# K-Kielak/dopamine

Measured on AMD Instinct MI355X. Metric: gradient-steps/sec (Rainbow, batch=32, 1M-transition buffer), higher is better.
Workload: dtype fp32; 1 GPU; Rainbow/C51 Asterix (9 actions), prioritized sum-tree replay, n=3, 1M-transition 84x84x4 uint8 buffer per GPU; global_batch=32, per_gpu_batch=32, replay_capacity=1000000, parallelism=dp1, hip_graph=True

## Files before the change

### dopamine_amd/csrc/nature_cnn.hip

```cpp
#include <algorithm>
#include <cassert>

#include "cnn_tile.h"
#include "c51_dev.h"

#include <cstring>
#include <optional>
#include <tuple>
#include <type_traits>

namespace dq {
namespace cnn {

constexpr int kGroupT = 1024;

template <int WM, int WN, int WK, class AL, class BL, class EP, bool kLate = true, int KS = 0,
          int NS = 0>
struct GemmOp {
  static constexpr int kT = 64 * WM * WN * WK;
  static constexpr bool kLateFetch = kLate;
  static constexpr int kLds = Tile<WM, WN, WK>::template lds<AL, BL>();
  AL a;
  BL b;
  EP e;
// ... 1240 lines not shown
  const int nc = std::max(kPubBlocks, blocks_for(P.lo, 2));
  const int na = blocks_for((P.n - P.lo) * (P.world - 1) / P.world, 4);
  auto rd = [&](int i) { return i >= 1 && i - 1 < n_riders ? riders + (i - 1) : nullptr; };
  launch(c, rd(1), b.dX_fc1());
  launch(c, rd(2), b.dW_fc1(), b.dX_c3(), b.dW_fc2());
  launch(c, rd(3), PeerPubOp{P, kPeerGrad}, b.dW_c3(), b.subpix_pairs(), b.dW_c2(), rs(s0, sm));
  launch(c, rd(4), b.sum_c3(), b.dW_c1(), rs(sm, s1));
  const PeerAgOp ag = defer_ag ? AgParts{&P, oa->var}.head()
                               : PeerAgOp{P, oa->var, na, 0, 0, INT64_MAX};
  launch(c, rd(5), PeerPubOp{P, kPeerParam}, b.sum_c2(), b.sum_c1(),
         P.world > 1 ? std::optional(ag) : std::nullopt);
  launch(c, NoRider{}, PeerExchOp{P, od, oa->var, oa->m, oa->v, nc}, head_layer<0>(head));
}

template <int kOpt>
void backward_head_from(Ctx& c, const dq_cnn_params* p, const dq_cnn_params* g, int B,
                        const float* x, const dq_cnn_acts* a, const float* dout, dq_cnn_acts* d,
                        const AdamHost& opt, int first, int last, const RiderDesc* r, int n_riders,
                        const FwdOps* hp, int head_from) {
  if (head_from == 7)
    backward_grouped<kOpt, 5>(c, p, g, B, x, a, dout, d, opt, first, last, r, n_riders, nullptr);
  else if (head_from == 6)
    backward_grouped<kOpt, 6>(c, p, g, B, x, a, dout, d, opt, first, last, r, n_riders, hp);
  else if (head_from == 5)
    backward_grouped<kOpt, 5>(c, p, g, B, x, a, dout, d, opt, first, last, r, n_riders, hp);
  else if (head_from == 4)
    backward_grouped<kOpt, 4>(c, p, g, B, x, a, dout, d, opt, first, last, r, n_riders, hp);
  else
    backward_grouped<kOpt>(c, p, g, B, x, a, dout, d, opt, first, last, r, n_riders, hp);
}

}
}

using namespace dq;
using namespace dq::cnn;

static int check_adam(const dq_cnn_params* p, const dq_cnn_params* g, const dq_adam_args* opt) {
  DQ_CHECK_ARG(opt->kind == DQ_OPT_ADAM || opt->kind == DQ_OPT_RMSPROP, "unknown optimizer kind");
  if (opt->kind == DQ_OPT_ADAM)
    DQ_CHECK_ARG(opt->var && opt->m && opt->v && opt->state && (opt->slot == 0 || opt->slot == 1),
                 "adam args: var, m, v, state and slot 0/1 required");
  else
    DQ_CHECK_ARG(opt->var && opt->m && opt->v && (!opt->centered || opt->mg),
                 "rmsprop args: var, ms (m), mom (v) and, centered, mg required");
  const float* w[10] = {p->conv1_w, p->conv1_b, p->conv2_w, p->conv2_b, p->conv3_w,
                        p->conv3_b, p->fc1_w,  p->fc1_b,  p->fc2_w,  p->fc2_b};
  const float* gw[10] = {g->conv1_w, g->conv1_b, g->conv2_w, g->conv2_b, g->conv3_w,
                         g->conv3_b, g->fc1_w,  g->fc1_b,  g->fc2_w,  g->fc2_b};
  for (int i = 0; i < 10; ++i) {
    DQ_CHECK_ARG(w[i] >= opt->var && (i == 0 || w[i] > w[i - 1]),
                 "parameters must live in the flat buffer opt->var in conv1..fc2 order");
    DQ_CHECK_ARG(gw[i] - g->conv1_w == w[i] - p->conv1_w,
                 "gradients must have the parameters' flat layout");
  }
  DQ_CHECK_ARG(((p->conv2_w - opt->var) & 3) == 0 && ((g->conv2_w - g->conv1_w) & 3) == 0,
               "16-byte aligned parameter views required");
  return DQ_OK;
}

#define DQ_TRY(expr)                   \
  do {                                 \
    const int rc_ = (expr);            \
    if (rc_ != DQ_OK) return rc_;      \
  } while (0)

static int check_net(bool args, int32_t batch, const dq_cnn_params* p, bool fc = true) {
  DQ_CHECK_ARG(args && batch >= 1, "null argument");
  DQ_CHECK_ARG(p->in_channels == 4 && (!fc || p->n_out >= 1),
               "the Nature CNN takes 84x84x4 NHWC input");
  return DQ_OK;
}
static int check_nets(bool args, int32_t batch, const dq_cnn_params* p0, const dq_cnn_params* p1,
                      const float* ws0, const float* ws1) {
  DQ_CHECK_ARG(args && batch >= 1, "null argument");
  DQ_CHECK_ARG(p0->in_channels == 4 && p1->in_channels == 4 && p0->n_out >= 1 && p1->n_out >= 1,
               "the Nature CNN takes 84x84x4 NHWC input");
  DQ_CHECK_ARG(ws0 != ws1, "the two networks need separate workspaces");
  return DQ_OK;
}
static int copy_riders(const dq_rider* riders, int32_t n_riders, int most, const char* too_many,
                       RiderDesc* r) {
  DQ_CHECK_ARG(0 <= n_riders && n_riders <= most && (riders || n_riders == 0), too_many);
  for (int i = 0; i < n_riders; ++i) {
    memcpy(&r[i], &riders[i], sizeof(RiderDesc));
    DQ_CHECK_ARG(r[i].kind >= kRiderNone && r[i].kind <= kRiderSetSample, "corrupt rider");
  }
  return DQ_OK;
}
static int head_ops(const dq_cnn_net* head, const float* ws, int32_t batch, FwdOps* hf,
                    const FwdOps** hp) {
  *hp = nullptr;
  if (!head) return DQ_OK;
  DQ_CHECK_ARG(head->p && head->x && head->a && head->ws, "null head network field");
  DQ_CHECK_ARG(head->p->in_channels == 4, "the Nature CNN takes 84x84x4 NHWC input");
  DQ_CHECK_ARG(head->ws != ws, "the head network needs its own workspace");
  *hf = FwdOps{head->p, head->x, head->a, head->ws, batch};
  *hp = hf;
  return DQ_OK;
}

static int check_peer(const dq_peer* peer, const float* var) {
  DQ_CHECK_ARG(peer && var, "null argument");
  const dq_peer& P = *peer;
  DQ_CHECK_ARG(P.world >= 1 && P.world <= DQ_PEER_MAX && P.rank >= 0 && P.rank < P.world,
               "peer: 1 <= world <= DQ_PEER_MAX, 0 <= rank < world");
  DQ_CHECK_ARG(P.lo >= 0 && P.lo % 4 == 0 && P.n > P.lo && (P.n - P.lo) % (4 * P.world) == 0,
               "peer: lo % 4 == 0 and (n - lo) % (4 world) == 0");
  DQ_CHECK_ARG(P.param[P.rank] == var, "peer: var must be this rank's parameter buffer");
  for (int q = 0; q < P.world; ++q)
    DQ_CHECK_ARG(P.grad[q] && P.param[q] && P.flags[q], "peer: null rank buffer");
  DQ_CHECK_ARG(P.max_polls > 0, "peer: max_polls must be positive");
  DQ_CHECK_ARG(P.xcds >= 0 && P.xcds <= 8, "peer: 0 <= xcds <= 8");
  return DQ_OK;
}

extern "C" {

int dq_cnn_forward(const dq_cnn_params* p, int32_t batch, const float* x, dq_cnn_acts* a,
                   float* ws, void* stream) {
  DQ_TRY(check_net(p && a && x && ws, batch, p));
  Ctx c{(hipStream_t)stream, ws, false, 0};
  forward(c, p, batch, x, a);
  DQ_CHECK_LAUNCH("dq_cnn_forward");
  return DQ_OK;
}

int dq_cnn_forward_pair(const dq_cnn_params* p0, const float* x0, dq_cnn_acts* a0, float* ws0,
                        const dq_cnn_params* p1, const float* x1, dq_cnn_acts* a1, float* ws1,
                        int32_t batch, void* stream) {
  DQ_TRY(check_nets(p0 && a0 && x0 && ws0 && p1 && a1 && x1 && ws1, batch, p0, p1, ws0, ws1));
  Ctx c0{(hipStream_t)stream, ws0, false, 0}, c1{(hipStream_t)stream, ws1, false, 0};
  forward_pair(c0, c1, p0, x0, a0, p1, x1, a1, batch);
  DQ_CHECK_LAUNCH("dq_cnn_forward_pair");
  return DQ_OK;
}

int dq_cnn_forward_head(const dq_cnn_params* p, int32_t batch, const float* x, dq_cnn_acts* a,
                        float* ws, void* stream) {
  DQ_TRY(check_net(p && a && x && ws, batch, p));
  Ctx c{(hipStream_t)stream, ws, false, 0};
  forward_head(c, FwdOps{p, x, a, ws, batch});
  DQ_CHECK_LAUNCH("dq_cnn_forward_head");
  return DQ_OK;
}

int dq_cnn_forward_with_tail(const dq_cnn_params* p0, const float* x0, dq_cnn_acts* a0, float* ws0,
                             const dq_cnn_params* p1, dq_cnn_acts* a1, float* ws1, int32_t batch,
                             void* stream) {
  DQ_TRY(check_nets(p0 && a0 && x0 && ws0 && p1 && a1 && ws1, batch, p0, p1, ws0, ws1));
  Ctx c0{(hipStream_t)stream, ws0, false, 0}, c1{(hipStream_t)stream, ws1, false, 0};
  forward_with_tail(c0, c1, FwdOps{p0, x0, a0, ws0, batch}, FwdOps{p1, nullptr, a1, ws1, batch});
  DQ_CHECK_LAUNCH("dq_cnn_forward_with_tail");
  return DQ_OK;
}

int dq_cnn_forward_fused(const dq_cnn_params* p0, const float* x0, dq_cnn_acts* a0, float* ws0,
                         const dq_cnn_params* p1, const float* x1, dq_cnn_acts* a1, float* ws1,
                         int32_t batch, int32_t fc1_1, void* stream) {
  DQ_TRY(check_nets(p0 && a0 && x0 && ws0 && p1 && a1 && ws1, batch, p0, p1, ws0, ws1));
  Ctx c0{(hipStream_t)stream, ws0, false, 0}, c1{(hipStream_t)stream, ws1, false, 0};
  DQ_CHECK_ARG((fc1_1 & 12) != 12, "flags 4 (convs only) and 8 (fc layers only) exclude each other");
  DQ_CHECK_ARG(!(fc1_1 & 32) || x1, "flag 32 (net 1's conv1) needs x1");
  forward_fused(c0, c1, FwdOps{p0, x0, a0, ws0, batch}, FwdOps{p1, x1, a1, ws1, batch},
                (fc1_1 & 1) != 0, (fc1_1 & 2) != 0, (fc1_1 & 8) == 0, (fc1_1 & 4) == 0,
                (fc1_1 & 16) != 0, (fc1_1 & 32) != 0);
  DQ_CHECK_LAUNCH("dq_cnn_forward_fused");
  return DQ_OK;
}

size_t dq_cnn_fc2_parts_offset(int32_t batch) { return FwdOps::part_offset(batch); }

int dq_cnn_forward_fused_c51(const dq_cnn_params* p0, const float* x0, dq_cnn_acts* a0, float* ws0,
                             const dq_cnn_params* p1, dq_cnn_acts* a1, float* ws1, int32_t batch,
                             const dq_c51_target* c51, int32_t flags, void* stream) {
  DQ_TRY(check_nets(p0 && a0 && x0 && ws0 && p1 && a1 && ws1 && c51, batch, p0, p1, ws0, ws1));
  DQ_CHECK_ARG((flags & 12) != 12, "flags 4 (convs only) and 8 (fc layers only) exclude each other");
  DQ_CHECK_ARG(c51->rewards && c51->terminals && c51->support && c51->m_out, "null C51 argument");
  DQ_CHECK_ARG(c51->num_atoms >= 2 && c51->num_atoms <= 64 && p1->n_out % c51->num_atoms == 0,
               "n_out must be num_actions * num_atoms, 2 <= num_atoms <= 64");
  const int A = p1->n_out / c51->num_atoms;
  DQ_CHECK_ARG(A <= 4 * kC51TgtMaxWaveRows, "the riding C51 target half takes at most 16 actions");
  Ctx c0{(hipStream_t)stream, ws0, false, 0}, c1{(hipStream_t)stream, ws1, false, 0};
  const FwdOps f0{p0, x0, a0, ws0, batch}, f1{p1, nullptr, a1, ws1, batch};
  const int NO = p1->n_out;
  C51Target t{LogitsParts{ws1 + FwdOps::part_offset(batch), p1->fc2_b, (int64_t)batch * NO,
                          FcHeadOp::kBands, NO},
              c51->rewards, c51->terminals, c51->support, batch, A, c51->num_atoms,
              c51->cumulative_gamma, c51->m_out, c51->target_logits_out};
  forward_fused_c51(c0, c1, f0, f1, t, (flags & 8) == 0, (flags & 4) == 0);
  DQ_CHECK_LAUNCH("dq_cnn_forward_fused_c51");
  return DQ_OK;
}


int dq_cnn_backward(const dq_cnn_params* p, const dq_cnn_params* g, int32_t batch, const float* x,
                    const dq_cnn_acts* a, const float* dout, dq_cnn_acts* d, float* ws,
                    void* stream) {
  DQ_TRY(check_net(p && g && a && d && x && dout && ws, batch, p));
  Ctx c{(hipStream_t)stream, ws, false, 0};
  backward_grouped<0>(c, p, g, batch, x, a, dout, d, AdamHost{nullptr});
  DQ_CHECK_LAUNCH("dq_cnn_backward");
  return DQ_OK;
}

int dq_cnn_backward_adam(const dq_cnn_params* p, const dq_cnn_params* g, int32_t batch,
                         const float* x, const dq_cnn_acts* a, const float* dout, dq_cnn_acts* d,
                         float* ws, const dq_adam_args* opt, void* stream) {
  DQ_TRY(check_net(p && g && a && d && x && dout && ws && opt, batch, p));
  DQ_TRY(check_adam(p, g, opt));
  Ctx c{(hipStream_t)stream, ws, false, 0};
  if (opt->kind == DQ_OPT_RMSPROP)
    backward_grouped<2>(c, p, g, batch, x, a, dout, d, AdamHost{opt});
  else
    backward_grouped<1>(c, p, g, batch, x, a, dout, d, AdamHost{opt});
  DQ_CHECK_LAUNCH("dq_cnn_backward_adam");
  return DQ_OK;
}

int dq_cnn_backward_groups(const dq_cnn_params* p, const dq_cnn_params* g, int32_t batch,
                           const float* x, const dq_cnn_acts* a, const float* dout,
                           dq_cnn_acts* d, float* ws, int32_t first, int32_t last, void* stream) {
  DQ_TRY(check_net(p && g && a && d && x && dout && ws, batch, p));
  DQ_CHECK_ARG(0 <= first && first <= last && last <= 7, "groups must satisfy 0 <= first <= last <= 7");
  Ctx c{(hipStream_t)stream, ws, false, 0};
  backward_grouped<0>(c, p, g, batch, x, a, dout, d, AdamHost{nullptr}, first, last);
  DQ_CHECK_LAUNCH("dq_cnn_backward_groups");
  return DQ_OK;
}

int dq_cnn_backward_riders(const dq_cnn_params* p, const dq_cnn_params* g, int32_t batch,
                           const float* x, const dq_cnn_acts* a, const float* dout,
                           dq_cnn_acts* d, float* ws, const dq_rider* riders, int32_t n_riders,
                           const dq_adam_args* opt, const dq_cnn_net* head, int32_t head_from,
                           int32_t first, int32_t last, void* stream) {
  DQ_TRY(check_net(p && g && a && d && x && dout && ws, batch, p));
  RiderDesc r[7];
  DQ_TRY(copy_riders(riders, n_riders, 7, "at most one rider per grouped launch (7)", r));
  DQ_CHECK_ARG(0 <= first && first <= last && last <= 7, "groups must satisfy 0 <= first <= last <= 7");
  DQ_CHECK_ARG(!opt || (first <= 1 && last == 7), "the fused optimizer needs the whole backward");
  DQ_CHECK_ARG(head_from >= 3 && head_from <= 7, "head_from must be in [3, 7]");
  FwdOps hf{};
  const FwdOps* hp;
  DQ_TRY(head_ops(head, ws, batch, &hf, &hp));
  Ctx c{(hipStream_t)stream, ws, false, 0};
  if (opt) {
    DQ_TRY(check_adam(p, g, opt));
    if (opt->kind == DQ_OPT_RMSPROP)
      backward_head_from<2>(c, p, g, batch, x, a, dout, d, AdamHost{opt}, first, last, r, n_riders,
                            hp, head_from);
    else
      backward_head_from<1>(c, p, g, batch, x, a, dout, d, AdamHost{opt}, first, last, r, n_riders,
                            hp, head_from);
  } else {
    backward_head_from<0>(c, p, g, batch, x, a, dout, d, AdamHost{nullptr}, first, last, r,
                          n_riders, hp, head_from);
  }
  DQ_CHECK_LAUNCH("dq_cnn_backward_riders");
  return DQ_OK;
}

int dq_cnn_backward_peer(const dq_cnn_params* p, const dq_cnn_params* g, int32_t batch,
                         const float* x, const dq_cnn_acts* a, const float* dout,
                         dq_cnn_acts* d, float* ws, const dq_rider* riders, int32_t n_riders,
                         const dq_adam_args* opt, const dq_cnn_net* head, const dq_peer* peer,
                         int32_t defer_ag, void* stream) {
  DQ_TRY(check_net(p && g && a && d && x && dout && ws && opt && peer, batch, p));
  DQ_CHECK_ARG(opt->kind == DQ_OPT_ADAM, "the peer exchange applies TF1 Adam");
  RiderDesc r[5];
  DQ_TRY(copy_riders(riders, n_riders, 5, "at most one rider per grouped launch 1..5", r));
  DQ_TRY(check_adam(p, g, opt));
  DQ_TRY(check_peer(peer, opt->var));
  const dq_peer& P = *peer;
  DQ_CHECK_ARG(P.n >= (int64_t)(p->fc2_b + p->n_out - opt->var),
               "peer: [lo, n) must reach the end of the flat parameter buffer");
  DQ_CHECK_ARG(P.lo == (int64_t)(p->fc1_w - opt->var),
               "peer: the sharded range is exactly the fc bucket [fc1_w, n) (pad the flat buffer "
               "so that its length divides into 4 world-float slices)");
  DQ_CHECK_ARG(P.param[P.rank] == opt->var && P.grad[P.rank] == g->conv1_w - (p->conv1_w - opt->var),
               "peer: this rank's buffers must be opt->var and the gradient of its layout");
  FwdOps hf{};
  const FwdOps* hp;
  DQ_TRY(head_ops(head, ws, batch, &hf, &hp));
  Ctx c{(hipStream_t)stream, ws, false, 0};
  backward_peer(c, p, g, batch, x, a, dout, d, opt, r, n_riders, hp, P, defer_ag != 0);
  DQ_CHECK_LAUNCH("dq_cnn_backward_peer");
  return DQ_OK;
}

int dq_peer_all_gather(const dq_peer* peer, float* var, void* stream) {
  DQ_TRY(check_peer(peer, var));
  const dq_peer& P = *peer;
  if (P.world > 1) {
    Ctx c{(hipStream_t)stream, nullptr, false, 0};
    group(c, AgParts{peer, var}.part(0), AgParts{peer, var}.part(1), AgParts{peer, var}.part(2));
  }
  DQ_CHECK_LAUNCH("dq_peer_all_gather");
  return DQ_OK;
}

#ifdef DQ_GROUP_PROF
int dq_debug_group_reset(void) {
  static unsigned z[dq::cnn::kGrpPos];
  return hipMemcpyToSymbol(HIP_SYMBOL(dq::cnn::g_grp_seq), z, sizeof(z)) == hipSuccess ? 0 : -1;
}
int dq_debug_peer_phases(void* recs, unsigned* seq) {
  if (hipMemcpyFromSymbol(seq, HIP_SYMBOL(dq::cnn::g_peer_ph_seq), sizeof(dq::cnn::g_peer_ph_seq)) !=
      hipSuccess)
    return -1;
  return hipMemcpyFromSymbol(recs, HIP_SYMBOL(dq::cnn::g_peer_ph), sizeof(dq::cnn::g_peer_ph)) ==
                 hipSuccess ? 0 : -1;
}
int dq_debug_group_read(void* recs, unsigned* seq, unsigned* dims) {
  dims[0] = dq::cnn::kGrpPos;
  dims[1] = dq::cnn::kGrpRing;
  if (hipMemcpyFromSymbol(seq, HIP_SYMBOL(dq::cnn::g_grp_seq), sizeof(dq::cnn::g_grp_seq)) !=
      hipSuccess)
    return -1;
  return hipMemcpyFromSymbol(recs, HIP_SYMBOL(dq::cnn::g_grp_rec), sizeof(dq::cnn::g_grp_rec)) ==
                 hipSuccess ? 0 : -1;
}
#endif

int dq_peer_selftest(const dq_peer* peer, uint32_t tag, int32_t* mismatches_out, void* stream) {
  DQ_CHECK_ARG(peer && mismatches_out, "null argument");
  const dq_peer& P = *peer;
  DQ_TRY(check_peer(peer, P.param[P.rank]));
  DQ_CHECK_ARG(P.n % 4 == 0 && P.n / 4 < (int64_t)1 << 27, "peer: n % 4 == 0, buffers < 2 GB");
  Ctx c{(hipStream_t)stream, nullptr, false, 0};
  group(c, SelfTestFillOp{P, tag, 2048});
  group(c, PeerPubOp{P, kPeerTest});
  group(c, SelfTestCheckOp{P, tag, mismatches_out, kPeerMaxBlocks});
  DQ_CHECK_LAUNCH("dq_peer_selftest");
  return DQ_OK;
}

int dq_cnn_forward_fused_peer(const dq_cnn_params* p0, const float* x0, dq_cnn_acts* a0, float* ws0,
                              const dq_cnn_params* p1, const float* x1, dq_cnn_acts* a1, float* ws1,
                              int32_t batch, int32_t fc1_1, const dq_peer* peer, float* var,
                              void* stream) {
  DQ_TRY(check_nets(p0 && a0 && x0 && ws0 && p1 && a1 && ws1, batch, p0, p1, ws0, ws1));
  DQ_CHECK_ARG((fc1_1 & (4 | 8 | 32)) == 0 && (fc1_1 & 16),
               "the deferred gather rides in the head_from 6 schedule's conv launches (flag 16)");
  DQ_TRY(check_peer(peer, var));
  Ctx c0{(hipStream_t)stream, ws0, false, 0}, c1{(hipStream_t)stream, ws1, false, 0};
  const AgParts ag{peer, var};
  forward_fused(c0, c1, FwdOps{p0, x0, a0, ws0, batch}, FwdOps{p1, x1, a1, ws1, batch},
                (fc1_1 & 1) != 0, (fc1_1 & 2) != 0, true, true, true, false,
                peer->world > 1 ? &ag : nullptr);
  DQ_CHECK_LAUNCH("dq_cnn_forward_fused_peer");
  return DQ_OK;
}

int dq_cnn_forward_torso(const dq_cnn_params* p, int32_t batch, const float* x, dq_cnn_acts* a,
                         float* ws, void* stream) {
  DQ_TRY(check_net(p && a && x && ws, batch, p, false));
  Ctx c{(hipStream_t)stream, ws, false, 0};
  const FwdOps f{p, x, a, ws, batch};
  group(c, f.conv1<false>());
  group(c, f.conv2<false>());
  group(c, f.conv3<false>());
  DQ_CHECK_LAUNCH("dq_cnn_forward_torso");
  return DQ_OK;
}

int dq_cnn_backward_torso(const dq_cnn_params* p, const dq_cnn_params* g, int32_t batch,
                          const float* x, const dq_cnn_acts* a, dq_cnn_acts* d, float* ws,
                          void* stream) {
  DQ_TRY(check_net(p && g && a && d && x && ws, batch, p, false));
  Ctx c{(hipStream_t)stream, ws, false, 0};
  backward_torso_grouped(c, p, g, batch, x, a, d);
  DQ_CHECK_LAUNCH("dq_cnn_backward_torso");
  return DQ_OK;
}

int dq_cnn_backward_torso_opt(const dq_cnn_params* p, const dq_cnn_params* g, int32_t batch,
                              const float* x, const dq_cnn_acts* a, dq_cnn_acts* d, float* ws,
                              const dq_adam_args* opt, float* head_begin, float* head_end,
                              void* stream) {
  DQ_TRY(check_net(p && g && a && d && x && ws && opt, batch, p, false));
  DQ_TRY(check_adam(p, g, opt));
  DQ_CHECK_ARG(head_begin && head_end && head_begin >= p->conv3_b + 64 && head_end > head_begin &&
                   ((head_begin - opt->var) & 3) == 0 && ((p->conv3_w - opt->var) & 3) == 0,
               "head range: 16-byte aligned, after conv3 in opt->var");
  Ctx c{(hipStream_t)stream, ws, false, 0};
  if (opt->kind == DQ_OPT_RMSPROP)
    backward_torso_grouped<2>(c, p, g, batch, x, a, d, AdamHost{opt}, head_begin, head_end);
  else
    backward_torso_grouped<1>(c, p, g, batch, x, a, d, AdamHost{opt}, head_begin, head_end);
  DQ_CHECK_LAUNCH("dq_cnn_backward_torso_opt");
  return DQ_OK;
}

int dq_cnn_backward_layer(const dq_cnn_params* p, const dq_cnn_params* g, int32_t batch,
                          const float* x, const dq_cnn_acts* a, const float* dout, dq_cnn_acts* d,
                          float* ws, int32_t layer, int32_t part, void* stream) {
  DQ_TRY(check_net(p && g && a && d && x && dout && ws, batch, p));
  Ctx c{(hipStream_t)stream, ws, false, 0};
  DQ_CHECK_ARG((part == 0 || part == 1) && backward_layer(c, p, g, batch, x, a, dout, d, layer, part),
               "layer must be 0..4 (fc2, fc1, conv3, conv2, conv1), part 0 (input grad, not conv1) "
               "or 1 (weight grad)");
  DQ_CHECK_LAUNCH("dq_cnn_backward_layer");
  return DQ_OK;
}

size_t dq_cnn_workspace_floats(int32_t batch, int32_t n_out) {
  dq_cnn_params p = {};
  dq_cnn_acts a = {};
  p.in_channels = 4;
  p.n_out = n_out;
  size_t need = 0;
  Ctx f{nullptr, nullptr, true, 0};
  forward(f, &p, batch, nullptr, &a);
  need = f.need > need ? f.need : need;
  for (int layer = 0; layer < 5; ++layer)
    for (int part = 0; part < 2; ++part) {
      Ctx l{nullptr, nullptr, true, 0};
      backward_layer(l, &p, &p, batch, nullptr, &a, nullptr, &a, layer, part);
      need = l.need > need ? l.need : need;
    }
  Ctx g{nullptr, nullptr, true, 0};
  backward_grouped<0>(g, &p, &p, batch, nullptr, &a, nullptr, &a, AdamHost{nullptr});
  need = g.need > need ? g.need : need;
  Ctx t{nullptr, nullptr, true, 0};
  backward_torso_grouped(t, &p, &p, batch, nullptr, &a, &a);
  need = t.need > need ? t.need : need;
  Ctx f0{nullptr, nullptr, true, 0}, f1{nullptr, nullptr, true, 0};
  forward_fused(f0, f1, FwdOps{&p, nullptr, &a, nullptr, batch}, FwdOps{&p, nullptr, &a, nullptr, batch},
                true);
  return f0.need > need ? f0.need : need;
}

}
```

### dopamine_amd/csrc/replay_dev.h

```cpp
#pragma once
#include "common.h"

namespace dq {

struct ReplayView {
  int64_t C;
  int64_t obs_bytes;
  int32_t S;
  int32_t n;
  int32_t depth;
  int32_t max_attempts;
  const uint8_t* frames;
  const int32_t* actions;
  const float* rewards;
  const uint8_t* terminals;
  double* tree;
  dq_replay_meta* meta;
  const uint32_t* tape;
  const float* discount;
};

__device__ __forceinline__ void latch(dq_replay_meta* m, int code, int arg, double val) {
  if (atomicCAS(&m->status, 0, code) == 0) {
    m->status_arg = arg;
// ... 432 lines not shown
  if (lane == 0) {
    if (L != v.n) {
      const int64_t nxt = pymod(idx + L, v.C);
      na = v.actions[nxt];
      nr = v.rewards[nxt];
    }
    if (g.action) g.action[b] = a0;
    if (g.reward) g.reward[b] = acc;
    if (g.next_action) g.next_action[b] = na;
    if (g.next_reward) g.next_reward[b] = nr;
    if (g.terminal) g.terminal[b] = term ? 1 : 0;
    if (g.indices_out) g.indices_out[b] = (int32_t)idx;
    if (g.probs) g.probs[b] = pr;
  }
}

__device__ inline void write_scalars_wave_short(const ReplayView& v, const GatherOut& g, int b,
                                          int64_t idx) {
  const int lane = threadIdx.x & 63;
  float p = 0.0f;
  bool t = false;
  const int64_t nspec = pymod(idx + v.n, v.C);
  int32_t a0 = 0, na = 0;
  float nr = 0.0f, pr = 0.0f;
  if (lane == 0) {
    a0 = v.actions[idx];
    na = v.actions[nspec];
    nr = v.rewards[nspec];
    if (g.probs) pr = (float)v.tree[((int64_t)1 << v.depth) - 1 + idx];
  }
  if (lane < v.n) {
    const int64_t j = pymod(idx + lane, v.C);
    t = v.terminals[j] != 0;
    p = __fmul_rn(v.discount[lane], v.rewards[j]);
  }
  const uint64_t tm = __ballot(t);
  int L = v.n;
  bool term = false;
  if (tm) {
    L = __ffsll((unsigned long long)tm);
    term = true;
  }
  float acc = 0.0f;
  for (int k = 0; k < L && k < kWave; ++k) acc = __fadd_rn(acc, __shfl(p, k));
  if (lane == 0) {
    if (v.n > kWave) {
      bool tt;
      L = traj_len(v, idx, &tt);
      term = tt;
      acc = 0.0f;
      for (int k = 0; k < L; ++k)
        acc = __fadd_rn(acc, __fmul_rn(v.discount[k], v.rewards[pymod(idx + k, v.C)]));
    }
    if (L != v.n) {
      const int64_t nxt = pymod(idx + L, v.C);
      na = v.actions[nxt];
      nr = v.rewards[nxt];
    }
    if (g.action) g.action[b] = a0;
    if (g.reward) g.reward[b] = acc;
    if (g.next_action) g.next_action[b] = na;
    if (g.next_reward) g.next_reward[b] = nr;
    if (g.terminal) g.terminal[b] = term ? 1 : 0;
    if (g.indices_out) g.indices_out[b] = (int32_t)idx;
    if (g.probs) g.probs[b] = pr;
  }
}

__device__ __forceinline__ float u8_unit(uint32_t x) {
  constexpr float kInv = 1.0f / 255.0f;
  const float xf = (float)x;
  const float q = __fmul_rn(xf, kInv);
  return __builtin_fmaf(__builtin_fmaf(-q, 255.0f, xf), kInv, q);
}

typedef uint32_t gather_u32x4 __attribute__((ext_vector_type(4)));

__device__ __forceinline__ float4 u8x4_to_f32_255(uint32_t w) {
  float4 o;
  o.x = u8_unit(w & 0xffu);
  o.y = u8_unit((w >> 8) & 0xffu);
  o.z = u8_unit((w >> 16) & 0xffu);
  o.w = u8_unit(w >> 24);
  return o;
}

enum { kScalEarly = 0, kScalLate = 1, kScalNone = 2 };

#ifdef DQ_GATHER_PROF
constexpr int kGpRing = 64, kGpWaves = 2048;
__device__ unsigned long long g_gp_wave[kGpRing][kGpWaves][4];
__device__ unsigned int g_gp_seq[kGpWaves];
#define GP_STAMP(gp, k)                                      \
  do {                                                       \
    asm volatile("s_waitcnt vmcnt(0)" ::: "memory");         \
    (gp)[k] = __builtin_amdgcn_s_memrealtime();              \
  } while (0)
#else
#define GP_STAMP(gp, k) do { } while (0)
#endif

template <int R, int kScalars = kScalEarly, bool kNt = false>
__device__ __forceinline__ void gather_nhwc4_body(const ReplayView& v, const GatherOut& g, int bx,
                                                  int slot, int tid,
                                                  unsigned long long* gp = nullptr) {
  constexpr bool kLateScalars = kScalars == kScalLate;
  const int b = slot >> 1, which = slot & 1;
  const bool scal = kScalars != kScalNone && bx == 0 && which == 0 && tid < 64;
  if (!kLateScalars && scal) write_scalars_wave_short(v, g, b, pymod((int64_t)g.indices[b], v.C));
  float* dst_base = (float*)(which ? g.next_state : g.state);
  const int64_t nd = v.obs_bytes >> 2;
  const int lane = tid & 63;
  const int64_t w0 = ((int64_t)bx * 256 + (tid & ~63)) * R;
  if (!dst_base || w0 >= nd) {
    if (kLateScalars && scal) write_scalars_wave_short(v, g, b, pymod((int64_t)g.indices[b], v.C));
    return;
  }
  const int64_t idx = pymod((int64_t)g.indices[b], v.C);
  if (gp) GP_STAMP(gp, 1);
  uint32_t w[R][4];
  auto load = [&](int64_t base) {
    const uint32_t* fr[4];
#pragma unroll
    for (int k = 0; k < 4; ++k)
      fr[k] = (const uint32_t*)(v.frames + pymod(base - 3 + k, v.C) * v.obs_bytes);
#pragma unroll
    for (int r = 0; r < R; ++r) {
      const int64_t d = w0 + 64 * r + lane;
#pragma unroll
      for (int k = 0; k < 4; ++k) w[r][k] = d < nd ? fr[k][d] : 0u;
    }
  };
  if (which) {
    const int64_t spec = pymod(idx + v.n, v.C);
    load(spec);
    bool term;
    const int64_t base = pymod(idx + traj_len_par(v, idx, &term), v.C);
    if (base != spec) load(base);
  } else {
    load(idx);
    if (kLateScalars && scal) write_scalars_wave_short(v, g, b, idx);
  }
  if (gp) GP_STAMP(gp, 2);
  const int sh = 8 * (lane & 3);
#pragma unroll
  for (int r = 0; r < R; ++r) {
    const int64_t d0 = w0 + 64 * r;
    float4* dst = (float4*)(dst_base + (int64_t)b * 4 * v.obs_bytes) + 4 * d0;
#pragma unroll
    for (int j = 0; j < 4; ++j) {
      const int src = 16 * j + (lane >> 2);
      float4 o;
      o.x = u8_unit((__shfl(w[r][0], src) >> sh) & 0xffu);
      o.y = u8_unit((__shfl(w[r][1], src) >> sh) & 0xffu);
      o.z = u8_unit((__shfl(w[r][2], src) >> sh) & 0xffu);
      o.w = u8_unit((__shfl(w[r][3], src) >> sh) & 0xffu);
      if (4 * d0 + 64 * j + lane < 4 * nd) {
        if constexpr (kNt)
          __builtin_amdgcn_raw_buffer_store_b128(
              *(const gather_u32x4*)&o, __builtin_amdgcn_make_buffer_rsrc(dst, 0, 0x7fffffff, 0x00020000),
              (64 * j + lane) * 16, 0, 2);
        else
          dst[64 * j + lane] = o;
      }
    }
  }
}

constexpr int kNhwcR = 1;

struct SetArgs {
  const int32_t* indices;
  const float* values;
  int64_t n;
  const double* values64;
};

__device__ __forceinline__ int readlane_i(int x, int l) { return __builtin_amdgcn_readlane(x, l); }
__device__ __forceinline__ double readlane_d(double x, int l) {
  const int lo = __builtin_amdgcn_readlane(__double2loint(x), l);
  const int hi = __builtin_amdgcn_readlane(__double2hiint(x), l);
  return __hiloint2double(hi, lo);
}

__device__ __forceinline__ double node_chain(bool act, int prev, double tree_val, double& delta,
                                             bool leaf, double val) {
  bool done = act && prev < 0;
  double before = tree_val, after = 0.0;
  if (done) {
    if (leaf) delta = __dsub_rn(val, before);
    after = __dadd_rn(before, delta);
  }
  while (__ballot(act && !done)) {
    const int src = prev < 0 ? 0 : prev;
    const double ap = __shfl(after, src);
    const int dp = __shfl((int)done, src);
    if (act && !done && dp) {
      before = ap;
      if (leaf) delta = __dsub_rn(val, before);
      after = __dadd_rn(before, delta);
      done = true;
    }
  }
  return after;
}

constexpr int kSumtreeParLds = kWave * 8;

template <int T>
__device__ inline void sumtree_set_par(const ReplayView& v, const SetArgs& a, void* lds) {
  constexpr int NW = T / 64;
  double* s_delta = (double*)lds;
  const int lane = threadIdx.x & 63, wave = threadIdx.x >> 6;
  dq_replay_meta* meta = v.meta;
  const int64_t l0 = a.n > 0 ? (lane < a.n ? lane : a.n - 1) : 0;
  const int32_t pre_i = (a.indices && a.n > 0) ? a.indices[l0] : 0;
  const double pre_v = a.n > 0 ? (a.values64 ? a.values64[l0] : (double)a.values[l0]) : 0.0;
  if (meta->status != 0) return;
  const int depth = v.depth;
  const int64_t base = meta->add_count;
  double maxrec = meta->max_recorded_priority;
  bool stop = false;
  for (int64_t c0 = 0; c0 < a.n && !stop; c0 += kWave) {
    const int m = (int)((a.n - c0) < kWave ? (a.n - c0) : kWave);
    int64_t idx = 0;
    double val = 0.0;
    if (lane < m) {
      if (c0 == 0) {
        idx = a.indices ? (int64_t)pre_i : pymod(base + lane, v.C);
        val = pre_v;
      } else {
        idx = a.indices ? (int64_t)a.indices[c0 + lane] : pymod(base + c0 + lane, v.C);
        val = a.values64 ? a.values64[c0 + lane] : (double)a.values[c0 + lane];
      }
    }
    const bool badi = lane < m && (idx < 0 || idx >= ((int64_t)1 << depth));
    const uint64_t negm = __ballot(lane < m && (val < 0.0 || badi));
    int me = m;
    if (negm) {
      me = __ffsll((unsigned long long)negm) - 1;
      stop = true;
    }
    const bool act = lane < me;
    if (wave == 0)
      for (int i = 0; i < me; ++i) {
        const double x = readlane_d(val, i);
        maxrec = (maxrec > x) ? maxrec : x;
      }
    const int node_leaf = act ? (int)idx : 0;
    auto links = [&](int L, int& prev, bool& last) {
      const int node = node_leaf >> (depth - L);
      prev = -1;
      last = true;
      for (int j = 0; j < me; ++j) {
        const int nj = readlane_i(node_leaf, j) >> (depth - L);
        if (nj == node) {
          if (j < lane) prev = j;
          if (j > lane) last = false;
        }
      }
    };
    constexpr int KL = (64 + NW - 1) / NW;
    double tv[KL];
#pragma unroll
    for (int k = 0; k < KL; ++k) {
      const int L = wave + NW * k;
      tv[k] = (act && L <= depth) ? v.tree[((int64_t)1 << L) - 1 + (node_leaf >> (depth - L))] : 0.0;
    }
    if (wave == depth % NW) {
      int prev;
      bool last;
      links(depth, prev, last);
      double delta = 0.0;
      node_chain(act, prev, tv[depth / NW], delta, true, val);
      if (act) s_delta[lane] = delta;
    }
    __syncthreads();
    double delta = act ? s_delta[lane] : 0.0;
#pragma unroll
    for (int k = 0; k < KL; ++k) {
      const int L = wave + NW * k;
      if (L > depth) break;
      int prev;
      bool last;
      links(L, prev, last);
      const double after = node_chain(act, prev, tv[k], delta, false, val);
      if (act && last) v.tree[((int64_t)1 << L) - 1 + (node_leaf >> (depth - L))] = after;
    }
    if (stop) {
      const int64_t bi = (int64_t)readlane_i((int)idx, me);
      const double bv = readlane_d(val, me);
      const bool oob = bi < 0 || bi >= ((int64_t)1 << depth);
      if (threadIdx.x == 0)
        latch(meta, oob ? DQ_ST_BAD_INDEX : DQ_ST_NEG_PRIORITY, (int)(c0 + me),
              oob ? (double)bi : bv);
    }
    __threadfence_block();
    __syncthreads();
  }
  if (threadIdx.x == 0) meta->max_recorded_priority = maxrec;
}

constexpr int kTopLevels = 11;
constexpr int kPerSampleParLds = kPerSampleLds + ((1 << kTopLevels) - 1) * 8;

template <int T>
__device__ inline void per_sample_par(const ReplayView& v, int B, int32_t* out, void* lds) {
  static_assert(T % 32 == 0, "32-lane groups");
  static_assert(kPerSampleLds % 8 == 0, "s_top alignment");
  int64_t* s_idx = (int64_t*)lds;
  uint8_t* s_ok = (uint8_t*)(s_idx + kMaxBatch);
  double* s_top = (double*)((uint8_t*)lds + kPerSampleLds);
  const int t = threadIdx.x, g = t >> 5, j = t & 31;
  dq_replay_meta* meta = v.meta;
  const int ktop = v.depth + 1 < kTopLevels ? v.depth + 1 : kTopLevels;
  const int ntop = (1 << ktop) - 1;
  constexpr int kTopR = ((1 << kTopLevels) - 1 + T - 1) / T;
  double top[kTopR];
#pragma unroll
  for (int r = 0; r < kTopR; ++r) top[r] = v.tree[min(t + r * T, ntop - 1)];
  const int64_t add_count = meta->add_count;
  const int64_t pos0 = meta->tape_pos;
  const int64_t len = meta->tape_len;
  const double total = v.tree[0];
  bool fail = meta->status != 0;
  if (!fail && total == 0.0) {
    if (t == 0) latch(meta, DQ_ST_EMPTY_TREE, 0, 0.0);
    fail = true;
  }
  if (!fail && pos0 + 2 * (int64_t)B > len) {
    if (t == 0) latch(meta, DQ_ST_TAPE_EXHAUSTED, 0, 0.0);
    fail = true;
  }
  if (fail) {
    if (t == 0) meta->reserved[0] = pos0;
    for (int i = t; i < B; i += T) out[i] = 0;
    return;
  }
#pragma unroll
  for (int r = 0; r < kTopR; ++r)
    if (t + r * T < ntop) s_top[t + r * T] = top[r];
  __syncthreads();
  const int l = 31 - __clz(j + 1), p = j + 1 - (1 << l);
  const double step = 1.0 / (double)B;
  for (int i0 = 0; i0 < B; i0 += T / 32) {
    const int i = i0 + g;
    const bool mine = i < B;
    double q = 0.0;
    if (mine) {
      const double u = res53(v.tape[pos0 + 2 * i], v.tape[pos0 + 2 * i + 1]);
      const double lo = __dmul_rn((double)i, step);
      const double hi = (i + 1 == B) ? 1.0 : __dmul_rn((double)(i + 1), step);
      q = __dmul_rn(__dadd_rn(lo, __dmul_rn(__dsub_rn(hi, lo), u)), total);
    }
    int64_t node = 0;
    for (int d = 0; d < ktop - 1; ++d) {
      const double lf = s_top[(2 << d) - 1 + 2 * node];
      if (q < lf) {
        node = 2 * node;
      } else {
        node = 2 * node + 1;
        q = __dsub_rn(q, lf);
      }
    }
    for (int d = ktop - 1; d < v.depth; d += 5) {
      const int lv = d + l + 1;
      double left = 0.0;
      if (mine && j < 31 && lv <= v.depth)
        left = v.tree[((int64_t)1 << lv) - 1 + 2 * ((node << l) + p)];
      int64_t pc = 0;
#pragma unroll
      for (int s = 0; s < 5; ++s) {
        if (d + s >= v.depth) break;
        const double lf = __shfl(left, (int)((1 << s) - 1 + pc), 32);
        if (q < lf) {
          pc = 2 * pc;
        } else {
          pc = 2 * pc + 1;
          q = __dsub_rn(q, lf);
        }
      }
      const int levels = v.depth - d < 5 ? v.depth - d : 5;
      node = (node << levels) + pc;
    }
    if (mine && j == 0) {
      s_idx[i] = node;
      s_ok[i] = is_valid(v, node, add_count);
    }
  }
  __syncthreads();
  if (t == 0) {
    int64_t pos = pos0 + 2 * (int64_t)B;
    int budget = v.max_attempts;
    for (int i = 0; i < B; ++i) {
      if (s_ok[i]) continue;
      if (budget == 0) {
        latch(meta, DQ_ST_MAX_ATTEMPTS, i, 0.0);
        break;
      }
      int64_t cand = s_idx[i];
      bool tape_dry = false;
      while (budget > 0) {
        if (pos + 2 > len) {
          tape_dry = true;
          break;
        }
        const double u = res53(v.tape[pos], v.tape[pos + 1]);
        pos += 2;
        cand = descend(v.tree, v.depth, __dmul_rn(u, total));
        --budget;
        if (is_valid(v, cand, add_count)) break;
      }
      s_idx[i] = cand;
      if (tape_dry) {
        latch(meta, DQ_ST_TAPE_EXHAUSTED, i, 0.0);
        break;
      }
    }
    meta->reserved[0] = pos0;
    meta->tape_pos = pos;
  }
  __syncthreads();
  for (int i = t; i < B; i += T) out[i] = (int32_t)s_idx[i];
}

enum RiderKind : int32_t { kRiderNone = 0, kRiderSet = 1, kRiderPerSample = 2,
                           kRiderUniformSample = 3, kRiderGatherNhwc = 4, kRiderSetSample = 5 };

struct RiderDesc {
  int32_t kind;
  int32_t batch;
  int32_t gx;
  int32_t groups;
  ReplayView v;
  GatherOut g;
  SetArgs s;
  int32_t* out;
};
static_assert(sizeof(RiderDesc) <= sizeof(dq_rider), "dq_rider too small");

constexpr int kRiderLds = kSumtreeParLds > kPerSampleParLds ? kSumtreeParLds : kPerSampleParLds;

template <int T, bool kGroups = false>
__device__ __forceinline__ void run_rider(const RiderDesc& r, int blk, void* lds) {
  static_assert(T % 256 == 0, "rider blocks are whole 256-thread gather sub-blocks");
  const int t = threadIdx.x;
  switch (r.kind) {
    case kRiderSet:
      sumtree_set_par<T>(r.v, r.s, lds);
      return;
    case kRiderPerSample:
      per_sample_par<T>(r.v, r.batch, r.out, lds);
      return;
    case kRiderSetSample:
      sumtree_set_par<T>(r.v, r.s, lds);
      __threadfence_block();
      __syncthreads();
      per_sample_par<T>(r.v, r.batch, r.out, lds);
      return;
    case kRiderUniformSample:
      if (t < kWave) {
        if constexpr (kGroups)
          uniform_sample_groups(r.v, r.batch, r.out, r.groups > 1 ? r.groups : 1);
        else
          uniform_sample_body(r.v, r.batch, r.out);
      }
      return;
    case kRiderGatherNhwc: {
      const int sub = blk * (T / 256) + t / 256;
      const int slot = sub / r.gx;
      if (slot < 2 * r.batch) gather_nhwc4_body<kNhwcR>(r.v, r.g, sub - slot * r.gx, slot, t & 255);
      return;
    }
    default:
      return;
  }
}

template <int T>
inline int rider_blocks(const RiderDesc& r) {
  if (r.kind == kRiderGatherNhwc) return (r.gx * 2 * r.batch + T / 256 - 1) / (T / 256);
  return r.kind == kRiderNone ? 0 : 1;
}

}
```

Measured before the change: 8347 gradient-steps/s.

## Parallelize prioritized-sample rejection retries across lane groups with wave-wide validity checks

Replaces the single-thread serial retry loop for invalid prioritized samples with a block-wide scheme. Each round draws one candidate per 32-lane group from the tape, and the candidates are then consumed in order so tape position and budget semantics stay the same as before. Validity checking is now spread across lanes, with terminal bytes checked in parallel and combined by ballot. The goal is to remove the serialized thread-0 descend and validity latency, at the cost of extra LDS, added barriers and more complex control flow; optional profiling stamps are also added.

```diff
diff --git a/dopamine_amd/csrc/nature_cnn.hip b/dopamine_amd/csrc/nature_cnn.hip
--- a/dopamine_amd/csrc/nature_cnn.hip
+++ b/dopamine_amd/csrc/nature_cnn.hip
@@ -1566,7 +1566,12 @@
 #ifdef DQ_GROUP_PROF
 int dq_debug_group_reset(void) {
   static unsigned z[dq::cnn::kGrpPos];
+  if (hipMemcpyToSymbol(HIP_SYMBOL(dq::g_ps_seq), z, sizeof(unsigned)) != hipSuccess) return -1;
   return hipMemcpyToSymbol(HIP_SYMBOL(dq::cnn::g_grp_seq), z, sizeof(z)) == hipSuccess ? 0 : -1;
+}
+int dq_debug_per_phases(void* recs, unsigned* seq) {
+  if (hipMemcpyFromSymbol(seq, HIP_SYMBOL(dq::g_ps_seq), sizeof(unsigned)) != hipSuccess) return -1;
+  return hipMemcpyFromSymbol(recs, HIP_SYMBOL(dq::g_ps_ph), sizeof(dq::g_ps_ph)) == hipSuccess ? 0 : -1;
 }
 int dq_debug_peer_phases(void* recs, unsigned* seq) {
   if (hipMemcpyFromSymbol(seq, HIP_SYMBOL(dq::cnn::g_peer_ph_seq), sizeof(dq::cnn::g_peer_ph_seq)) !=
diff --git a/dopamine_amd/csrc/replay_dev.h b/dopamine_amd/csrc/replay_dev.h
--- a/dopamine_amd/csrc/replay_dev.h
+++ b/dopamine_amd/csrc/replay_dev.h
@@ -758,17 +758,72 @@
 }
 
 constexpr int kTopLevels = 11;
-constexpr int kPerSampleParLds = kPerSampleLds + ((1 << kTopLevels) - 1) * 8;
+constexpr int kPerCand = 32;
+constexpr int kPerSampleParLds =
+    kPerSampleLds + ((1 << kTopLevels) - 1) * 8 + kPerCand * 8 + kPerCand;
+
+#ifdef DQ_GROUP_PROF
+constexpr int kPsRing = 128, kPsPhases = 9;
+static __device__ unsigned long long g_ps_ph[kPsRing][kPsPhases];
+static __device__ unsigned int g_ps_seq;
+#define PS_STAMP(k)                                          \
+  do {                                                       \
+    asm volatile("s_waitcnt vmcnt(0)" ::: "memory");         \
+    if (threadIdx.x == 0) g_ps_ph[ps][k] = __builtin_amdgcn_s_memrealtime(); \
+  } while (0)
+#else
+#define PS_STAMP(k) do { } while (0)
+#endif
+
+__device__ __forceinline__ int64_t wrap1(int64_t a, int64_t C) {
+  return a < 0 ? a + C : (a >= C ? a - C : a);
+}
+__device__ __forceinline__ bool is_valid_group(const ReplayView& v, int64_t idx, int64_t add_count,
+                                               int64_t cursor, int j) {
+  auto byte = [&](int k) {
+    const int64_t at = wrap1(idx - v.S + 1 + min(k, v.S - 2), v.C);
+    return v.terminals[max((int64_t)0, min(at, v.C - 1))] != 0;
+  };
+  bool term = byte(j) && v.S > 1;
+  if (v.S - 1 > 32) {
+#pragma clang loop unroll(disable) vectorize(disable) interleave(disable)
+    for (int k0 = 32; k0 < v.S - 1; k0 += 32) term |= byte(k0 + j);
+  }
+  const uint32_t any = (uint32_t)(__ballot(term) >> (threadIdx.x & 32));
+  if (idx >= v.C) return false;
+  if (add_count < v.C && (idx >= cursor - v.n || idx < v.S - 1)) return false;
+  if (wrap1(idx - (cursor - v.n), v.C) < (int64_t)(v.n + v.S)) return false;
+  return any == 0;
+}
+
+__device__ __forceinline__ int per_next_invalid(const uint8_t* s_ok, int from, int B) {
+  const int lane = threadIdx.x & 63;
+#pragma clang loop unroll(disable) vectorize(disable) interleave(disable)
+  for (int b0 = from & ~63; b0 < B; b0 += kWave) {
+    const int i = b0 + lane;
+    const uint64_t m = __ballot(i >= from && i < B && s_ok[min(i, B - 1)] == 0);
+    if (m) return b0 + __ffsll((unsigned long long)m) - 1;
+  }
+  return -1;
+}
 
 template <int T>
 __device__ inline void per_sample_par(const ReplayView& v, int B, int32_t* out, void* lds) {
-  static_assert(T % 32 == 0, "32-lane groups");
+  constexpr int NG = T / 32;
+  static_assert(T % 64 == 0 && NG <= kPerCand, "32-lane groups, whole waves");
   static_assert(kPerSampleLds % 8 == 0, "s_top alignment");
   int64_t* s_idx = (int64_t*)lds;
   uint8_t* s_ok = (uint8_t*)(s_idx + kMaxBatch);
   double* s_top = (double*)((uint8_t*)lds + kPerSampleLds);
+  int64_t* s_cidx = (int64_t*)(s_top + (1 << kTopLevels) - 1);
+  uint8_t* s_cok = (uint8_t*)(s_cidx + kPerCand);
   const int t = threadIdx.x, g = t >> 5, j = t & 31;
   dq_replay_meta* meta = v.meta;
+#ifdef DQ_GROUP_PROF
+  const unsigned ps = g_ps_seq % kPsRing;
+  if (t == 0) g_ps_ph[ps][0] = __builtin_amdgcn_s_memrealtime();
+  else if (t < kPsPhases) g_ps_ph[ps][t] = 0;
+#endif
   const int ktop = v.depth + 1 < kTopLevels ? v.depth + 1 : kTopLevels;
   const int ntop = (1 << ktop) - 1;
   constexpr int kTopR = ((1 << kTopLevels) - 1 + T - 1) / T;
@@ -797,18 +852,26 @@
   for (int r = 0; r < kTopR; ++r)
     if (t + r * T < ntop) s_top[t + r * T] = top[r];
   __syncthreads();
+  PS_STAMP(1);
   const int l = 31 - __clz(j + 1), p = j + 1 - (1 << l);
   const double step = 1.0 / (double)B;
-  for (int i0 = 0; i0 < B; i0 += T / 32) {
+  const int64_t cursor = add_count % v.C;
+  int64_t pos = pos0 + 2 * (int64_t)B;
+  int budget = v.max_attempts;
+  int open = -1, scan = 0;
+  bool cand = false;
+  for (int i0 = 0;;) {
     const int i = i0 + g;
-    const bool mine = i < B;
+    const bool mine = cand ? (g < budget && pos + 2 * (int64_t)g + 2 <= len) : i < B;
     double q = 0.0;
     if (mine) {
-      const double u = res53(v.tape[pos0 + 2 * i], v.tape[pos0 + 2 * i + 1]);
-      const double lo = __dmul_rn((double)i, step);
-      const double hi = (i + 1 == B) ? 1.0 : __dmul_rn((double)(i + 1), step);
+      const int64_t at = cand ? pos + 2 * (int64_t)g : pos0 + 2 * (int64_t)i;
+      const double u = res53(v.tape[at], v.tape[at + 1]);
+      const double lo = cand ? 0.0 : __dmul_rn((double)i, step);
+      const double hi = (cand || i + 1 == B) ? 1.0 : __dmul_rn((double)(i + 1), step);
       q = __dmul_rn(__dadd_rn(lo, __dmul_rn(__dsub_rn(hi, lo), u)), total);
     }
+    if (!cand && i0 == 0) PS_STAMP(2);
     int64_t node = 0;
     for (int d = 0; d < ktop - 1; ++d) {
       const double lf = s_top[(2 << d) - 1 + 2 * node];
@@ -819,6 +882,7 @@
         q = __dsub_rn(q, lf);
       }
     }
+    if (!cand && i0 == 0) PS_STAMP(3);
     for (int d = ktop - 1; d < v.depth; d += 5) {
       const int lv = d + l + 1;
       double left = 0.0;
@@ -838,46 +902,74 @@
       }
       const int levels = v.depth - d < 5 ? v.depth - d : 5;
       node = (node << levels) + pc;
-    }
-    if (mine && j == 0) {
-      s_idx[i] = node;
-      s_ok[i] = is_valid(v, node, add_count);
-    }
-  }
-  __syncthreads();
-  if (t == 0) {
-    int64_t pos = pos0 + 2 * (int64_t)B;
-    int budget = v.max_attempts;
-    for (int i = 0; i < B; ++i) {
-      if (s_ok[i]) continue;
-      if (budget == 0) {
-        latch(meta, DQ_ST_MAX_ATTEMPTS, i, 0.0);
-        break;
-      }
-      int64_t cand = s_idx[i];
-      bool tape_dry = false;
-      while (budget > 0) {
-        if (pos + 2 > len) {
-          tape_dry = true;
+#ifdef DQ_GROUP_PROF
+      if (!cand && i0 == 0 && d < ktop + 9) PS_STAMP(d == ktop - 1 ? 4 : 5);
+#endif
+    }
+    const bool ok = is_valid_group(v, node, add_count, cursor, j);
+    if (!cand) {
+      if (mine && j == 0) {
+        s_idx[i] = node;
+        s_ok[i] = ok;
+      }
+      i0 += NG;
+      if (i0 < B) continue;
+      PS_STAMP(6);
+    } else if (j == 0) {
+      s_cidx[g] = node;
+      s_cok[g] = ok;
+    }
+    __syncthreads();
+    const int have = cand ? NG : 0;
+    int c = 0;
+    bool more = false;
+    for (;;) {
+      if (open < 0) {
+        open = per_next_invalid(s_ok, scan, B);
+        if (open < 0) break;
+        if (budget == 0) {
+          if (t == 0) latch(meta, DQ_ST_MAX_ATTEMPTS, open, 0.0);
           break;
         }
-        const double u = res53(v.tape[pos], v.tape[pos + 1]);
-        pos += 2;
-        cand = descend(v.tree, v.depth, __dmul_rn(u, total));
-        --budget;
-        if (is_valid(v, cand, add_count)) break;
-      }
-      s_idx[i] = cand;
-      if (tape_dry) {
-        latch(meta, DQ_ST_TAPE_EXHAUSTED, i, 0.0);
+      }
+      if (budget == 0) {
+        scan = open + 1;
+        open = -1;
+        continue;
+      }
+      if (pos + 2 > len) {
+        if (t == 0) latch(meta, DQ_ST_TAPE_EXHAUSTED, open, 0.0);
         break;
       }
-    }
+      if (c == have) {
+        more = true;
+        break;
+      }
+      if (t == 0) s_idx[open] = s_cidx[c];
+      const bool okc = __builtin_amdgcn_readfirstlane((int)s_cok[c]) != 0;
+      pos += 2;
+      --budget;
+      ++c;
+      if (okc) {
+        scan = open + 1;
+        open = -1;
+      }
+    }
+    if (!more) break;
+    cand = true;
+    __syncthreads();
+  }
+  PS_STAMP(7);
+  if (t == 0) {
     meta->reserved[0] = pos0;
     meta->tape_pos = pos;
   }
   __syncthreads();
   for (int i = t; i < B; i += T) out[i] = (int32_t)s_idx[i];
+#ifdef DQ_GROUP_PROF
+  PS_STAMP(8);
+  if (t == 0) g_ps_seq = g_ps_seq + 1;
+#endif
 }
 
 enum RiderKind : int32_t { kRiderNone = 0, kRiderSet = 1, kRiderPerSample = 2,
```

New measurement: 8428 gradient-steps/s, median of 6. About the same (+1.0%).
